# profi248/backuwup

Hardware: AMD Instinct MI355X
Metric: GB/s chunked+hashed+deduped (whole node, 1/2/4/8 GPU), bit-exact vs CPU (higher is better)
Workload: dtype u8

## Files before the change

backuwup_amd/csrc/bw_cdc.hip:

```cpp
#include "bw_device.h"
#include "bw_internal.h"

namespace bw {
#if BW_CLOCK_STAMPS
__device__ ClockLog* g_clk_cdc = nullptr;
void clock_log_register_cdc(void* log) { hipMemcpyToSymbol(HIP_SYMBOL(g_clk_cdc), &log, sizeof(log)); }
#endif


__constant__ uint64_t c_gear[256] = BW_GEAR_INIT;


__device__ __forceinline__ uint64_t gear_fetch(uint32_t word, uint32_t sel, uint32_t lane_off, const uint64_t* lds) {
    const uint32_t addr = __builtin_amdgcn_perm(word, lane_off, sel);
    return *(const uint64_t*)((const uint8_t*)lds + addr);
}

__device__ __forceinline__ void gear_step(uint64_t& h, uint32_t word, uint32_t sel, uint32_t lane_off,
                                          const uint64_t* lds) {
    h = (h << 1) + gear_fetch(word, sel, lane_off, lds);
}

#define BW_SEL(k) (0x0c0c0000u | ((4u + (k)) << 8))

__device__ __forceinline__ uint32_t mask_test(uint64_t h, uint32_t mlo, uint32_t mhi) {
    uint32_t r;
    const uint32_t t = (uint32_t)h & mlo;
    asm("v_and_or_b32 %0, %1, %2, %3" : "=v"(r) : "v"((uint32_t)(h >> 32)), "s"(mhi), "v"(t));
    return r;
}

__device__ __forceinline__ void record_hit(uint64_t pos, uint64_t h, const Masks& mk, uint32_t* s_cnt,
                                           uint64_t* s_slots) {
    const bool S = (h & mk.mask_s) == 0, L = (h & mk.mask_l) == 0;
    if (S || L) {
        uint32_t i = atomicAdd(s_cnt, 1u);
        if (i < (uint32_t)SCAN_CAP) s_slots[i] = pos | (S ? BW_CAND_S : 0) | (L ? BW_CAND_L : 0);
    }
}

__device__ __forceinline__ void hash_words(uint64_t& h, uint32_t& acc, const uint32_t (&ww)[16], uint32_t lane_off,
                                           const uint64_t* s_gear, uint32_t phi) {
#pragma unroll
    for (int i = 0; i < 16; i += 2) {
        uint64_t g[8];
#pragma unroll
        for (int q = 0; q < 8; q++) g[q] = gear_fetch(ww[i + q / 4], BW_SEL(q % 4), lane_off, s_gear);
#pragma unroll
        for (int q = 0; q < 8; q += 2) {
            h = (h << 1) + g[q];
            const uint32_t t0 = (uint32_t)(h >> 32) & phi;
            h = (h << 1) + g[q + 1];
            const uint32_t t1 = (uint32_t)(h >> 32) & phi;
            asm("v_min3_u32 %0, %1, %2, %3" : "=v"(acc) : "v"(acc), "v"(t0), "v"(t1));
        }
    }
}

__device__ __forceinline__ void stage_hash_step(uint4 r0, uint4 r1, uint4 r2, uint4 r3, uint8_t* wr,
                                                const uint8_t* rd, uint64_t& h, uint64_t at, uint32_t lane_off,
                                                const uint64_t* s_gear, uint32_t phi, uint32_t* cnt,
                                                uint64_t* slots) {
    *(uint4*)(wr) = r0;
    *(uint4*)(wr + 16 * STAGE_ROW) = r1;
    *(uint4*)(wr + 32 * STAGE_ROW) = r2;
    *(uint4*)(wr + 48 * STAGE_ROW) = r3;
    __builtin_amdgcn_wave_barrier();
    const uint4 v0 = *(const uint4*)(rd), v1 = *(const uint4*)(rd + 16), v2 = *(const uint4*)(rd + 32),
                v3 = *(const uint4*)(rd + 48);
    __builtin_amdgcn_wave_barrier();
    const uint32_t ww[16] = {v0.x, v0.y, v0.z, v0.w, v1.x, v1.y, v1.z, v1.w,
                             v2.x, v2.y, v2.z, v2.w, v3.x, v3.y, v3.z, v3.w};
    uint32_t acc = 0xffffffffu;
    hash_words(h, acc, ww, lane_off, s_gear, phi);
    if (__builtin_expect(acc == 0, 0)) {
        const uint32_t i = atomicAdd(cnt, 1u);
        if (i < (uint32_t)SCAN_CAP) slots[i] = at | BW_CAND_BLK;
    }
}

constexpr uint32_t TILE_OVF = 0x80000000u;

__device__ __forceinline__ void ovf_push(uint64_t t, uint32_t* ovf, uint64_t* ctr) {
    const uint64_t k = atomicAdd((unsigned long long*)&ctr[C_NOVF], 1ull);
    ovf[k] = (uint32_t)t;
}

__device__ __forceinline__ void refine_block(const uint8_t* __restrict__ data, uint64_t b, const uint64_t* s_gear,
                                             uint32_t lane, const Masks& mk, uint32_t* cnt, uint64_t* slots) {
    const uint32_t rep = (lane & 31) * 8;
    const uint64_t g0 = b >= 64 ? *(const uint64_t*)((const uint8_t*)s_gear + ((uint32_t)data[b - 64 + lane] << 8) + rep) : 0;
    const uint64_t g1 = *(const uint64_t*)((const uint8_t*)s_gear + ((uint32_t)data[b + lane] << 8) + rep);
    const uint64_t pre = bw_shfl64(bw_gear_scan(g0), 63);
    const uint64_t h = bw_gear_scan(g1) + ((pre << lane) << 1);
    record_hit(b + lane, h >> mk.pre_shift, mk, cnt, slots);
}


template <int BLOCK, int STRIP>
__global__ __launch_bounds__(BLOCK, 4) void k_scan(const uint8_t* __restrict__ data, uint64_t n_bytes,
                                                       uint64_t n_tiles, Masks mk,
                                                       uint32_t* __restrict__ tile_count,
                                                       uint64_t* __restrict__ tile_slots, uint32_t* __restrict__ ovf,
                                                       uint64_t* ctr) {
    constexpr int WAVES = BLOCK / 64;
    struct ScanLds {
        uint64_t gear[256 * GEAR_REP];
        uint8_t stage[WAVES][64 * STAGE_ROW];
        uint64_t slots[WAVES][SCAN_CAP];
        uint64_t flags[WAVES][SCAN_CAP];
        uint32_t cnt[WAVES], nflag[WAVES];
    };
    __shared__ __attribute__((aligned(16))) ScanLds lds;
    uint64_t* s_gear = lds.gear;
    uint8_t (*s_stage)[64 * STAGE_ROW] = lds.stage;
    uint64_t (*s_slots)[SCAN_CAP] = lds.slots;
    uint32_t* s_cnt = lds.cnt;
    for (int i = threadIdx.x; i < 256 * GEAR_REP; i += blockDim.x) s_gear[i] = c_gear[i / GEAR_REP] << mk.pre_shift;
    __syncthreads();
    const uint32_t lane = threadIdx.x & 63, wid = threadIdx.x >> 6;
    const uint32_t lane_off = (lane & 31) * 8;
    const uint32_t phi = mk.pre_hi;
    uint8_t* stage = s_stage[wid];
    uint32_t* cnt = &s_cnt[wid];
    uint64_t* slots = s_slots[wid];
    uint32_t* fcnt = &lds.nflag[wid];
    uint64_t* fslots = lds.flags[wid];
    const uint64_t nw = (uint64_t)gridDim.x * WAVES;

    for (uint64_t tile = (uint64_t)blockIdx.x * WAVES + wid; tile < n_tiles; tile += nw) {
#if BW_CLOCK_STAMPS
        ClockStamp clk((tile & 15) == 0 ? g_clk_cdc : nullptr, 0);
#endif
        if (lane == 0) { *cnt = 0; *fcnt = 0; }
        const uint64_t base = tile * (64ull * STRIP);
        const uint64_t ss = base + (uint64_t)lane * STRIP;
        uint64_t h = 0;
        if (base + (64ull * STRIP) <= n_bytes) {
            if (ss >= 64) {
                const uint4* wp = (const uint4*)(data + ss - 64);
                uint4 w[4];
#pragma unroll
                for (int i = 0; i < 4; i++) w[i] = wp[i];
#pragma unroll
                for (int i = 0; i < 4; i++) {
                    const uint32_t ww[4] = {w[i].x, w[i].y, w[i].z, w[i].w};
#pragma unroll
                    for (int j = 0; j < 4; j++)
#pragma unroll
                        for (int k = 0; k < 4; k++) gear_step(h, ww[j], BW_SEL(k), lane_off, s_gear);
                }
            }
            {
                const uint8_t* src = data + base + (uint64_t)(lane >> 2) * STRIP + (lane & 3) * 16;
                uint8_t* wr = stage + (lane >> 2) * STAGE_ROW + (lane & 3) * 16;
                const uint8_t* rd = stage + lane * STAGE_ROW;
                constexpr int STEPS = STRIP / SCAN_STEP;
                constexpr uint64_t JS = 16ull * STRIP;
#define BW_LOAD8(r, ds)                                                                          \
    do {                                                                                         \
        const uint8_t* s_ = src + (uint64_t)(ds) * (2 * SCAN_STEP);                              \
        _Pragma("unroll") for (int j = 0; j < 4; j++) {                                          \
            r[j] = *(const uint4*)(s_ + j * JS);                                                 \
            r[4 + j] = *(const uint4*)(s_ + SCAN_STEP + j * JS);                                 \
        }                                                                                        \
    } while (0)
                uint4 a[8], b[8];
                BW_LOAD8(a, 0);
#pragma unroll 1
                for (int ds = 0; ds < STEPS / 2; ds += 2) {
                    BW_LOAD8(b, ds + 1);
                    stage_hash_step(a[0], a[1], a[2], a[3], wr, rd, h, ss + (uint64_t)(2 * ds) * SCAN_STEP, lane_off,
                                    s_gear, phi, fcnt, fslots);
                    stage_hash_step(a[4], a[5], a[6], a[7], wr, rd, h, ss + (uint64_t)(2 * ds + 1) * SCAN_STEP,
                                    lane_off, s_gear, phi, fcnt, fslots);
                    BW_LOAD8(a, ds + 2 < STEPS / 2 ? ds + 2 : STEPS / 2 - 1);
                    stage_hash_step(b[0], b[1], b[2], b[3], wr, rd, h, ss + (uint64_t)(2 * ds + 2) * SCAN_STEP,
                                    lane_off, s_gear, phi, fcnt, fslots);
                    stage_hash_step(b[4], b[5], b[6], b[7], wr, rd, h, ss + (uint64_t)(2 * ds + 3) * SCAN_STEP,
                                    lane_off, s_gear, phi, fcnt, fslots);
                }
#undef BW_LOAD8
            }
        } else if (ss < n_bytes) {
            const uint64_t se = ss + STRIP < n_bytes ? ss + STRIP : n_bytes;
            for (uint64_t p = ss >= 64 ? ss - 64 : 0; p < se; p++) {
                h = (h << 1) + s_gear[(uint32_t)data[p] * GEAR_REP];
                if (p >= ss) record_hit(p, h >> mk.pre_shift, mk, cnt, slots);
            }
        }
        __builtin_amdgcn_wave_barrier();
        const uint32_t nf = __builtin_amdgcn_readfirstlane(*fcnt);
        if (nf <= (uint32_t)SCAN_CAP)
            for (uint32_t f = 0; f < nf; f++) refine_block(data, BW_CAND_POS(fslots[f]), s_gear, lane, mk, cnt, slots);
        __builtin_amdgcn_wave_barrier();
        if (lane == 0) {
            const uint32_t c = *cnt, n = c < (uint32_t)SCAN_CAP ? c : (uint32_t)SCAN_CAP;
            if (nf > (uint32_t)SCAN_CAP || c > (uint32_t)SCAN_CAP) ovf_push(tile, ovf, ctr);
            for (uint32_t i = 1; i < n; i++) {
                uint64_t v = slots[i];
                int k = (int)i - 1;
                while (k >= 0 && BW_CAND_POS(slots[k]) > BW_CAND_POS(v)) {
                    slots[k + 1] = slots[k];
                    k--;
                }
                slots[k + 1] = v;
            }
            tile_count[tile] = c;
            for (uint32_t i = 0; i < n; i++) tile_slots[tile * SCAN_CAP + i] = slots[i];
        }
        __builtin_amdgcn_wave_barrier();
    }
}

template <int BLOCK, int STRIP>
static void launch_scan_t(hipStream_t st, const uint8_t* data, uint64_t n_bytes, uint64_t n_tiles, const Masks& mk,
                          uint32_t* tile_count, uint64_t* tile_slots, uint32_t* ovf, uint64_t* ctr) {
    uint64_t grid = (n_tiles + BLOCK / 64 - 1) / (BLOCK / 64);
    const uint64_t cap = STRIP == SCAN_STRIP ? 512 : 1024;
    if (grid > cap) grid = cap;
    hipLaunchKernelGGL((k_scan<BLOCK, STRIP>), dim3((unsigned)grid), dim3(BLOCK), 0, st, data, n_bytes,
                       n_tiles, mk, tile_count, tile_slots, ovf, ctr);
}

bool launch_scan(hipStream_t st, const uint8_t* data, uint64_t n_bytes, uint64_t n_tiles, const Masks& mk,
                 uint32_t* tile_count, uint64_t* tile_slots, uint32_t* ovf, uint64_t* ctr, int waves) {
    if (!n_tiles) return true;
    const bool big = 64ull * SCAN_STRIP == 1ull << mk.tile_shift, small = 64ull * SCAN_STRIP_SMALL == 1ull << mk.tile_shift;
    if (!big && !small) return false;
#if BW_DIAG
    if (waves == 8) {
        if (big) launch_scan_t<512, SCAN_STRIP>(st, data, n_bytes, n_tiles, mk, tile_count, tile_slots, ovf, ctr);
        else launch_scan_t<512, SCAN_STRIP_SMALL>(st, data, n_bytes, n_tiles, mk, tile_count, tile_slots, ovf, ctr);
        return true;
    }
#endif
    (void)waves;
    if (big) launch_scan_t<SCAN_BLOCK, SCAN_STRIP>(st, data, n_bytes, n_tiles, mk, tile_count, tile_slots, ovf, ctr);
    else launch_scan_t<SCAN_BLOCK, SCAN_STRIP_SMALL>(st, data, n_bytes, n_tiles, mk, tile_count, tile_slots, ovf, ctr);
    return true;
}


template <int T>
__device__ __forceinline__ uint64_t block_excl_sum(uint64_t v, uint64_t* s, uint64_t* total) {
    s[threadIdx.x] = v;
    __syncthreads();
    for (int d = 1; d < T; d <<= 1) {
        uint64_t a = threadIdx.x >= (unsigned)d ? s[threadIdx.x - d] : 0;
        __syncthreads();
        s[threadIdx.x] += a;
        __syncthreads();
    }
    const uint64_t incl = s[threadIdx.x];
    if (total) *total = s[T - 1];
    __syncthreads();
    return incl - v;
}

template <int T>
__device__ __forceinline__ uint64_t block_excl_segmax(uint32_t f, uint64_t v, uint64_t* s, uint32_t* sf) {
    s[threadIdx.x] = v;
    sf[threadIdx.x] = f;
    __syncthreads();
    for (int d = 1; d < T; d <<= 1) {
        uint64_t a = 0;
        uint32_t af = 0;
        const bool has = threadIdx.x >= (unsigned)d;
        if (has) { a = s[threadIdx.x - d]; af = sf[threadIdx.x - d]; }
        __syncthreads();
        if (has && !sf[threadIdx.x]) { s[threadIdx.x] = a > s[threadIdx.x] ? a : s[threadIdx.x]; sf[threadIdx.x] = af; }
        __syncthreads();
    }
    uint64_t r = (threadIdx.x > 0) ? s[threadIdx.x - 1] : 0;
    __syncthreads();
    return r;
}

__device__ __forceinline__ bool last_block_done(uint64_t* done) {
    __shared__ bool last;
    __syncthreads();
    if (threadIdx.x == 0) {
        __threadfence();
        last = atomicAdd((unsigned long long*)done, 1ull) == gridDim.x - 1;
    }
    __syncthreads();
    if (last) {
        __threadfence();
        if (threadIdx.x == 0) *done = 0;
    }
    return last;
}

template <int T>
__device__ __forceinline__ uint64_t scan_totals(uint64_t* tot, uint64_t n, uint64_t* s) {
    const uint64_t per = (n + T - 1) / T, lo = threadIdx.x * per;
    const uint64_t hi = lo + per < n ? lo + per : n;
    uint64_t sum = 0;
    for (uint64_t i = lo; i < hi; i++) sum += tot[i];
    uint64_t total;
    uint64_t run = block_excl_sum<T>(sum, s, &total);
    for (uint64_t i = lo; i < hi; i++) {
        const uint64_t t = tot[i];
        tot[i] = run;
        run += t;
    }
    return total;
}


constexpr int BLK = 1024;

constexpr int RESCAN_THREADS = 256;

template <bool WRITE>
__device__ uint64_t rescan_tile(const uint8_t* __restrict__ data, uint64_t n_bytes, const Masks& mk, uint64_t tile,
                                uint64_t base, uint64_t* __restrict__ cand, uint64_t cap, const uint64_t* s_gear,
                                uint64_t* s_scan) {
    const uint64_t rs = (1ull << mk.tile_shift) / RESCAN_THREADS;
    const uint64_t ss = (tile << mk.tile_shift) + (uint64_t)threadIdx.x * rs;
    const uint64_t se = ss + rs < n_bytes ? ss + rs : n_bytes;
    uint64_t mine = 0, total = 0;
    for (int pass = 0; pass < (WRITE ? 2 : 1); pass++) {
        uint64_t h = 0, w = 0;
        if (pass == 1) w = base + block_excl_sum<RESCAN_THREADS>(mine, s_scan, nullptr);
        if (ss < n_bytes) {
            for (uint64_t p = ss >= 64 ? ss - 64 : 0; p < se; p++) {
                h = (h << 1) + s_gear[data[p]];
                if (p < ss) continue;
                const bool S = (h & mk.mask_s) == 0, L = (h & mk.mask_l) == 0;
                if (S || L) {
                    if (pass == 0) mine++;
                    else if (w < cap) cand[w++] = p | (S ? BW_CAND_S : 0) | (L ? BW_CAND_L : 0);
                }
            }
        }
    }
    if (!WRITE) block_excl_sum<RESCAN_THREADS>(mine, s_scan, &total);
    __syncthreads();
    return total;
}

template <bool WRITE>
__device__ void rescan_range(const uint8_t* __restrict__ data, uint64_t n_bytes, const Masks& mk,
                             const uint32_t* __restrict__ ovf, uint64_t novf, uint64_t t0, uint64_t t1,
                             uint32_t* __restrict__ tile_count, const uint64_t* __restrict__ off,
                             uint64_t* __restrict__ cand, uint64_t cap, uint64_t* s_gear, uint64_t* s_scan) {
    bool loaded = false;
    for (uint64_t k = 0; k < novf; k++) {
        const uint64_t tile = ovf[k];
        if (tile < t0 || tile >= t1) continue;
        if (!loaded) {
            for (int i = threadIdx.x; i < 256; i += blockDim.x) s_gear[i] = c_gear[i];
            __syncthreads();
            loaded = true;
        }
        const uint64_t total = rescan_tile<WRITE>(data, n_bytes, mk, tile, WRITE ? off[tile] : 0, cand, cap, s_gear,
                                                  s_scan);
        if (!WRITE && threadIdx.x == 0) tile_count[tile] = (uint32_t)total | TILE_OVF;
    }
    __syncthreads();
}

constexpr int TS_BLOCK = 256;

template <bool WRITE>
__global__ __launch_bounds__(RESCAN_THREADS) void k_rescan(const uint8_t* __restrict__ data, uint64_t n_bytes, Masks mk,
                                                            const uint32_t* __restrict__ ovf, uint32_t* __restrict__ cnt,
                                                            const uint64_t* __restrict__ off, uint64_t* __restrict__ cand,
                                                            uint64_t cap, const uint64_t* ctr) {
    __shared__ uint64_t s_gear[256], s_scan[RESCAN_THREADS];
    const uint64_t novf = ctr[C_NOVF];
    if (blockIdx.x >= novf) return;
    for (int i = threadIdx.x; i < 256; i += blockDim.x) s_gear[i] = c_gear[i];
    __syncthreads();
    for (uint64_t k = blockIdx.x; k < novf; k += gridDim.x) {
        const uint64_t tile = ovf[k];
        const uint64_t total = rescan_tile<WRITE>(data, n_bytes, mk, tile, WRITE ? off[tile] : 0, cand, cap, s_gear, s_scan);
        if (!WRITE && threadIdx.x == 0) cnt[tile] = (uint32_t)total | TILE_OVF;
    }
}

__global__ __launch_bounds__(TS_BLOCK) void k_tile_partial(const uint8_t* __restrict__ data, uint64_t n_bytes, Masks mk,
                                                           const uint32_t* __restrict__ ovf, uint32_t* __restrict__ cnt,
                                                           uint64_t n, uint64_t* __restrict__ off,
                                                           uint64_t* __restrict__ btot, uint64_t cap, uint64_t* ctr,
                                                           bool spread) {
    __shared__ uint64_t s[TS_BLOCK];
    __shared__ uint64_t s_gear[256];
    const uint64_t novf = spread ? 0 : ctr[C_NOVF];
    if (novf) {
        const uint64_t t0 = (uint64_t)blockIdx.x * 4 * TS_BLOCK, t1 = t0 + 4 * TS_BLOCK;
        rescan_range<false>(data, n_bytes, mk, ovf, novf, t0, t1 < n ? t1 : n, cnt, nullptr, nullptr, 0, s_gear, s);
    }
    const uint64_t i0 = ((uint64_t)blockIdx.x * TS_BLOCK + threadIdx.x) * 4;
    uint32_t c[4] = {0, 0, 0, 0};
    if (i0 + 4 <= n) {
        const uint4 v = *(const uint4*)(cnt + i0);
        c[0] = v.x; c[1] = v.y; c[2] = v.z; c[3] = v.w;
    } else {
        for (int k = 0; k < 4; k++) c[k] = i0 + k < n ? cnt[i0 + k] : 0;
    }
    for (int k = 0; k < 4; k++) c[k] &= ~TILE_OVF;
    const uint64_t sum = (uint64_t)c[0] + c[1] + c[2] + c[3];
    uint64_t total;
    uint64_t run = block_excl_sum<TS_BLOCK>(sum, s, &total);
    for (int k = 0; k < 4; k++)
        if (i0 + k < n) { off[i0 + k] = run; run += c[k]; }
    if (threadIdx.x == 0) btot[blockIdx.x] = total;
    if (!last_block_done(&ctr[C_DONE_TILES])) return;
    const uint64_t all = scan_totals<TS_BLOCK>(btot, gridDim.x, s);
    if (threadIdx.x == 0) {
        off[n] = all;
        ctr[C_NCAND] = all < cap ? all : cap;
        ctr[C_CANDTOTAL] = all;
        ctr[C_TRUNC] = BW_NONE;
    }
}

__global__ __launch_bounds__(256) void k_compact(const uint8_t* __restrict__ data, uint64_t n_bytes, Masks mk,
                                                 const uint32_t* __restrict__ ovf, const uint32_t* __restrict__ cnt,
                                                 const uint64_t* __restrict__ slots, uint64_t* __restrict__ off,
                                                 const uint64_t* __restrict__ bbase, uint64_t n_tiles,
                                                 uint64_t* __restrict__ cand, uint64_t cap, uint64_t* ctr, bool spread) {
    const uint64_t t = (uint64_t)blockIdx.x * blockDim.x + threadIdx.x;
    if (t < n_tiles) {
        const uint64_t o = off[t] + bbase[t / (4 * TS_BLOCK)];
        off[t] = o;
        const uint32_t c = cnt[t];
        if (o + (c & ~TILE_OVF) > cap)
            atomicMin((unsigned long long*)&ctr[C_TRUNC], (unsigned long long)(t << mk.tile_shift));
        if (!(c & TILE_OVF)) {
            for (uint32_t i = 0; i < c; i++)
                if (o + i < cap) cand[o + i] = slots[t * SCAN_CAP + i];
        }
    }
    const uint64_t novf = spread ? 0 : ctr[C_NOVF];
    if (novf) {
        __shared__ uint64_t s_gear[256], s_scan[RESCAN_THREADS];
        __syncthreads();
        const uint64_t t0 = (uint64_t)blockIdx.x * blockDim.x, t1 = t0 + blockDim.x;
        rescan_range<true>(data, n_bytes, mk, ovf, novf, t0, t1 < n_tiles ? t1 : n_tiles, nullptr, off, cand, cap,
                           s_gear, s_scan);
    }
}

void launch_compact(hipStream_t st, const uint8_t* data, uint64_t n_bytes, uint64_t n_tiles, const Masks& mk,
                    uint32_t* tile_count, uint64_t* tile_slots, uint64_t* tile_off, uint64_t* cand,
                    uint64_t cand_cap, uint32_t* ovf_list, uint64_t* ctr, uint64_t* btot) {
    if (!n_tiles) return;
    const uint64_t nb = (n_tiles + 4 * TS_BLOCK - 1) / (4 * TS_BLOCK);
    const double flagged = (double)(1ull << mk.tile_shift) / 64.0 *
                           (1.0 - pow(1.0 - ldexp(1.0, -__builtin_popcount(mk.pre_hi)), 64.0));
    const bool spread = flagged > SCAN_CAP / 2;
    const unsigned rb = (unsigned)std::min<uint64_t>(n_tiles, 2048);
    if (spread)
        hipLaunchKernelGGL(k_rescan<false>, dim3(rb), dim3(RESCAN_THREADS), 0, st, data, n_bytes, mk, ovf_list, tile_count,
                           nullptr, nullptr, 0, ctr);
    hipLaunchKernelGGL(k_tile_partial, dim3((unsigned)nb), dim3(TS_BLOCK), 0, st, data, n_bytes, mk, ovf_list,
                       tile_count, n_tiles, tile_off, btot, cand_cap, ctr, spread);
    hipLaunchKernelGGL(k_compact, dim3((unsigned)((n_tiles + 255) / 256)), dim3(256), 0, st, data, n_bytes, mk, ovf_list,
                       tile_count, tile_slots, tile_off, btot, n_tiles, cand, cand_cap, ctr, spread);
    if (spread)
        hipLaunchKernelGGL(k_rescan<true>, dim3(rb), dim3(RESCAN_THREADS), 0, st, data, n_bytes, mk, ovf_list, tile_count,
                           tile_off, cand, cand_cap, ctr);
}


struct Walker {
    const uint8_t* data;
    const uint64_t* cand;
    uint64_t ncand;
    const uint64_t* lgear;
    Masks mk;
    uint64_t trunc;
    uint64_t data_len;
};

__device__ uint64_t direct_scan(const Walker& W, uint64_t a, uint64_t hi, uint64_t c2a) {
    const int lane = bw_lane();
    BW_ASSERT(a >= 64 && a <= hi && hi <= W.data_len);
    uint64_t carry = bw_shfl64(bw_gear_scan(W.lgear[W.data[a - 64 + lane]]), 63);
    for (uint64_t b = a; b < hi; b += 64) {
        const uint64_t p = b + (uint64_t)lane;
        const bool valid = p < hi;
        const uint64_t g = valid ? W.lgear[W.data[p]] : 0;
        const uint64_t h = bw_gear_scan(g) + ((carry << lane) << 1);
        const uint64_t mask = p < c2a ? W.mk.mask_s : W.mk.mask_l;
        const uint64_t hb = __ballot(valid && (h & mask) == 0);
        if (hb) return b + (uint64_t)__builtin_ctzll(hb);
        carry = bw_shfl64(h, 63);
    }
    return BW_NONE;
}

__device__ uint64_t walk_next(const Walker& W, uint64_t s, uint64_t fe, uint64_t& cptr) {
    const int lane = bw_lane();
    BW_ASSERT(s < fe && fe <= W.data_len);
    const uint64_t rem = fe - s;
    if (rem <= W.mk.min) return fe;
    uint64_t center = W.mk.avg, remaining = rem;
    if (rem > W.mk.max) remaining = W.mk.max;
    else if (rem < center) center = rem;
    const uint64_t s0 = W.mk.s0, c2 = center & ~1ull, r2 = remaining & ~1ull;

    const uint64_t p = s0 + (uint64_t)lane;
    const bool valid = lane < 47 && p < r2;
    const uint64_t g = valid ? W.lgear[W.data[s + p]] : 0;
    const uint64_t h = bw_gear_scan(g);
    const uint64_t mask = p < c2 ? W.mk.mask_s : W.mk.mask_l;
    const uint64_t hb = __ballot(valid && (h & mask) == 0);
    if (hb) return s + s0 + (uint64_t)__builtin_ctzll(hb);

    const uint64_t lo = s + s0 + 47, hi = s + r2, c2a = s + c2;
    const uint64_t hc = hi < W.trunc ? hi : W.trunc;
    for (;;) {
        const uint64_t idx = cptr + (uint64_t)lane;
        const uint64_t c = idx < W.ncand ? W.cand[idx] : BW_NONE;
        const uint64_t pos = c == BW_NONE ? BW_NONE : BW_CAND_POS(c);
        const uint64_t below = __ballot(pos < lo);
        const bool match = pos >= lo && pos < hc && ((pos < c2a) ? (c & BW_CAND_S) != 0 : (c & BW_CAND_L) != 0);
        const uint64_t mb = __ballot(match);
        if (mb) {
            const uint64_t cut = bw_shfl64(pos, __builtin_ctzll(mb));
            cptr += (uint64_t)__popcll(below);
            BW_ASSERT(cut > s && cut < s + remaining && cptr <= W.ncand + 64);
            return cut;
        }
        if (__ballot(pos >= hc) != 0) {
            cptr += (uint64_t)__popcll(below);
            break;
        }
        cptr += 64;
    }
    if (hc < hi) {
        const uint64_t cut = direct_scan(W, lo > hc ? lo : hc, hi, c2a);
        if (cut != BW_NONE) return cut;
    }
    return s + remaining;
}

__device__ __forceinline__ void load_lgear(uint64_t* lg) {
    for (int i = threadIdx.x; i < 256; i += blockDim.x) lg[i] = c_gear[i];
    __syncthreads();
}


constexpr int WAVES_PER_BLOCK = 4;

__global__ __launch_bounds__(64 * WAVES_PER_BLOCK) void k_chains(Walker W, const uint64_t* __restrict__ tile_off,
                                                                 const uint64_t* ctr, const SegDesc* __restrict__ segs,
                                                                 uint64_t nseg, uint64_t* __restrict__ chains,
                                                                 uint32_t* __restrict__ chain_n,
                                                                 uint64_t* __restrict__ chain_cptr) {
    __shared__ uint64_t lg[256];
    load_lgear(lg);
    W.lgear = lg;
    W.ncand = ctr[C_NCAND];
    W.trunc = ctr[C_TRUNC];
    const uint64_t j = (uint64_t)blockIdx.x * WAVES_PER_BLOCK + threadIdx.x / 64;
    if (j >= nseg) return;
    const SegDesc sd = segs[j];
    uint64_t s = sd.start, cptr = tile_off[s >> W.mk.tile_shift];
    uint32_t n = 0;
    bool past = false;
    for (;;) {
        const uint64_t c = walk_next(W, s, sd.file_end, cptr);
        if (n < (uint32_t)CHAIN_CAP && bw_lane() == 0) chains[j * CHAIN_CAP + n] = c;
        n++;
        if (n > (uint32_t)CHAIN_CAP || c >= sd.file_end || (c >= sd.end && past)) break;
        past = c >= sd.end;
        s = c;
    }
    if (bw_lane() == 0) { chain_n[j] = n; chain_cptr[j] = cptr; }
}

__global__ __launch_bounds__(64 * WAVES_PER_BLOCK) void k_extend(Walker W, const uint64_t* ctr,
                                                                 const SegDesc* __restrict__ segs, uint64_t nseg,
                                                                 uint64_t* __restrict__ chains,
                                                                 uint32_t* __restrict__ chain_n,
                                                                 const uint64_t* __restrict__ chain_cptr,
                                                                 uint64_t* __restrict__ merge) {
    __shared__ uint64_t lg[256];
    load_lgear(lg);
    W.lgear = lg;
    W.ncand = ctr[C_NCAND];
    W.trunc = ctr[C_TRUNC];
    const uint64_t j = (uint64_t)blockIdx.x * WAVES_PER_BLOCK + threadIdx.x / 64;
    if (j >= nseg) return;
    const int lane = bw_lane();
    const SegDesc sd = segs[j];
    if (sd.last) { if (lane == 0) merge[j] = sd.file_end; return; }
    uint32_t n = chain_n[j];
    const uint32_t n1r = chain_n[j + 1];
    if (n > (uint32_t)CHAIN_CAP || n1r == 0) { if (lane == 0) merge[j] = BW_NONE; return; }
    const uint32_t n1 = n1r < (uint32_t)CHAIN_CAP ? n1r : (uint32_t)CHAIN_CAP;
    const uint64_t* c1 = chains + (j + 1) * CHAIN_CAP;
    const uint64_t v0 = (uint32_t)lane < n1 ? c1[lane] : BW_NONE;
    const uint64_t v1 = (uint32_t)lane + 64 < n1 ? c1[lane + 64] : BW_NONE;
    const uint64_t last1 = c1[n1 - 1];
    const uint64_t b1 = segs[j + 1].start;
    uint64_t e = chains[j * CHAIN_CAP + n - 1], cptr = chain_cptr[j], m = BW_NONE;
    for (;;) {
        if (e == b1 || __ballot(v0 == e || v1 == e) != 0) { m = e; break; }
        if (e >= last1 || n >= (uint32_t)CHAIN_CAP) break;
        e = walk_next(W, e, sd.file_end, cptr);
        if (lane == 0) chains[j * CHAIN_CAP + n] = e;
        n++;
    }
    if (lane == 0) { chain_n[j] = n; merge[j] = m; }
}

void launch_chains(hipStream_t st, const uint8_t* data, uint64_t data_len, const Masks& mk, const uint64_t* cand,
                   const uint64_t* tile_off, uint64_t* ctr, const SegDesc* segs, uint64_t nseg, uint64_t* chains,
                   uint32_t* chain_n, uint64_t* chain_cptr, uint64_t* merge, int force_serial) {
    if (!nseg || force_serial) return;
    Walker W{data, cand, 0, nullptr, mk, 0, data_len};
    const unsigned grid = (unsigned)((nseg + WAVES_PER_BLOCK - 1) / WAVES_PER_BLOCK);
    hipLaunchKernelGGL(k_chains, dim3(grid), dim3(64 * WAVES_PER_BLOCK), 0, st, W, tile_off, ctr, segs, nseg,
                       chains, chain_n, chain_cptr);
    hipLaunchKernelGGL(k_extend, dim3(grid), dim3(64 * WAVES_PER_BLOCK), 0, st, W, ctr, segs, nseg, chains,
                       chain_n, chain_cptr, merge);
}


__global__ __launch_bounds__(BLK) void k_resolve(const SegDesc* __restrict__ segs, uint64_t nseg,
                                                 const CFileDesc* __restrict__ cfiles, uint64_t ncf,
                                                 const uint64_t* __restrict__ chains,
                                                 const uint32_t* __restrict__ chain_n,
                                                 const uint64_t* __restrict__ merge, uint64_t* __restrict__ seg_M,
                                                 uint32_t* __restrict__ seg_cnt, uint32_t* __restrict__ cf_invalid,
                                                 int force_serial) {
    __shared__ uint64_t s_v[BLK];
    __shared__ uint32_t s_f[BLK];
    for (uint64_t f = threadIdx.x; f < ncf; f += BLK) cf_invalid[f] = 0;
    __syncthreads();
    const uint64_t per = (nseg + BLK - 1) / BLK, lo = threadIdx.x * per;
    const uint64_t hi = lo + per < nseg ? lo + per : nseg;
    uint32_t af = 0;
    uint64_t av = 0;
    for (uint64_t j = lo; j < hi; j++) {
        const bool head = cfiles[segs[j].cfile].first_seg == j;
        const uint64_t m = merge[j];
        if (head) { af = 1; av = m; } else { av = m > av ? m : av; }
    }
    uint64_t run = block_excl_segmax<BLK>(af, av, s_v, s_f);
    for (uint64_t j = lo; j < hi; j++) {
        const SegDesc sd = segs[j];
        const bool head = cfiles[sd.cfile].first_seg == j;
        if (head) run = 0;
        const uint64_t M = head ? sd.start : run;
        seg_M[j] = M;
        const uint64_t m = merge[j];
        run = m > run ? m : run;
        if (force_serial) { cf_invalid[sd.cfile] = 1; continue; }
    }
    __syncthreads();
    if (force_serial) return;
    for (uint64_t j = lo; j < hi; j++) {
        const SegDesc sd = segs[j];
        const uint32_t nr = chain_n[j];
        const uint64_t M = seg_M[j];
        const uint64_t R = sd.last ? sd.file_end : seg_M[j + 1];
        bool ok = nr <= (uint32_t)CHAIN_CAP && M != BW_NONE && R != BW_NONE;
        uint32_t cnt = 0;
        if (ok) {
            bool found = (M == sd.start);
            cnt = (M == sd.start && sd.start < R) ? 1 : 0;
            for (uint32_t k = 0; k < nr; k++) {
                const uint64_t e = chains[j * CHAIN_CAP + k];
                if (e == M) found = true;
                if (e >= M && e < R && e != sd.start) cnt++;
            }
            if (!sd.last && R > M) {
                bool reach = false;
                for (uint32_t k = 0; k < nr; k++) reach |= chains[j * CHAIN_CAP + k] == R;
                ok = reach;
            }
            ok = ok && found;
        }
        seg_cnt[j] = cnt;
        if (!ok) cf_invalid[sd.cfile] = 1;
    }
}

__global__ __launch_bounds__(64 * WAVES_PER_BLOCK) void k_fallback(Walker W, const uint64_t* __restrict__ tile_off,
                                                                   uint64_t* ctr, const CFileDesc* __restrict__ cfiles,
                                                                   uint64_t ncf, const uint32_t* __restrict__ cf_invalid,
                                                                   uint64_t* __restrict__ fb_starts,
                                                                   uint64_t* __restrict__ fb_count) {
    __shared__ uint64_t lg[256];
    load_lgear(lg);
    W.lgear = lg;
    W.ncand = ctr[C_NCAND];
    W.trunc = ctr[C_TRUNC];
    const uint64_t f = (uint64_t)blockIdx.x * WAVES_PER_BLOCK + threadIdx.x / 64;
    if (f >= ncf || !cf_invalid[f]) return;
    const CFileDesc cf = cfiles[f];
    uint64_t s = cf.start, cptr = tile_off[s >> W.mk.tile_shift], n = 0;
    while (s < cf.end) {
        if (bw_lane() == 0) fb_starts[cf.fb_off + n] = s;
        n++;
        s = walk_next(W, s, cf.end, cptr);
    }
    if (bw_lane() == 0) {
        fb_count[f] = n;
        atomicAdd((unsigned long long*)&ctr[C_NINVALID], 1ull);
    }
}

void launch_resolve(hipStream_t st, const uint8_t* data, uint64_t data_len, const Masks& mk, const uint64_t* cand,
                    const uint64_t* tile_off, uint64_t* ctr, const SegDesc* segs, uint64_t nseg,
                    const CFileDesc* cfiles, uint64_t ncf, const uint64_t* chains, const uint32_t* chain_n,
                    const uint64_t* merge, uint64_t* seg_M, uint32_t* seg_cnt, uint32_t* cf_invalid,
                    uint64_t* fb_starts, uint64_t* fb_count, int force_serial) {
    if (!nseg) return;
    hipLaunchKernelGGL(k_resolve, dim3(1), dim3(BLK), 0, st, segs, nseg, cfiles, ncf, chains, chain_n, merge, seg_M,
                       seg_cnt, cf_invalid, force_serial);
    Walker W{data, cand, 0, nullptr, mk, 0, data_len};
    const unsigned grid = (unsigned)((ncf + WAVES_PER_BLOCK - 1) / WAVES_PER_BLOCK);
    hipLaunchKernelGGL(k_fallback, dim3(grid), dim3(64 * WAVES_PER_BLOCK), 0, st, W, tile_off, ctr, cfiles, ncf,
                       cf_invalid, fb_starts, fb_count);
}


__device__ __forceinline__ uint64_t groups_of(uint64_t len, uint32_t gshift) {
    const uint64_t leaves = len == 0 ? 1 : (len + B3_LEAF_BYTES - 1) / B3_LEAF_BYTES;
    return (leaves + (1u << gshift) - 1) >> gshift;
}

template <bool WRITE>
__device__ void unit_blobs(const UnitDesc& u, const SegDesc* segs, const CFileDesc* cfiles, const uint64_t* chains,
                           const uint32_t* chain_n, const uint64_t* seg_M, const uint32_t* cf_invalid,
                           const uint64_t* fb_starts, const uint64_t* fb_count, BlobArrays b, uint64_t bbase,
                           uint64_t gbase, uint64_t& nb, uint64_t& ng) {
    nb = 0;
    ng = 0;
    auto emit = [&](uint64_t start, uint64_t end, uint32_t kind, uint64_t fend) {
        const uint64_t len = end - start;
        BW_ASSERT(start <= end && end <= fend && fend <= b.data_len);
        if (WRITE) {
            const uint64_t k = bbase + nb;
            BW_ASSERT(k < b.cap);
            b.start[k] = start;
            b.len[k] = len;
            b.goff[k] = gbase + ng;
            b.file[k] = u.file;
            b.kind[k] = kind;
            b.fend[k] = fend;
        }
        nb++;
        ng += groups_of(len, b.gshift);
    };
    if (u.kind == 0) { emit(u.start, u.start + u.len, 0, u.start + u.len); return; }
    const SegDesc sd = segs[u.seg];
    if (cf_invalid[u.cfile]) {
        const CFileDesc cf = cfiles[u.cfile];
        if (cf.first_seg != u.seg) return;
        const uint64_t n = fb_count[u.cfile];
        for (uint64_t i = 0; i < n; i++) {
            const uint64_t s = fb_starts[cf.fb_off + i];
            const uint64_t e = i + 1 < n ? fb_starts[cf.fb_off + i + 1] : cf.end;
            emit(s, e, 1, cf.end);
        }
        return;
    }
    const uint64_t M = seg_M[u.seg];
    const uint64_t R = sd.last ? sd.file_end : seg_M[u.seg + 1];
    if (M >= R) return;
    const uint32_t nr = chain_n[u.seg];
    uint64_t prev = BW_NONE;
    if (M == sd.start) prev = sd.start;
    for (uint32_t k = 0; k < nr; k++) {
        const uint64_t e = chains[u.seg * CHAIN_CAP + k];
        if (e < M || e == sd.start) continue;
        if (e >= R) break;
        if (prev != BW_NONE) emit(prev, e, 1, sd.file_end);
        prev = e;
    }
    if (prev != BW_NONE) emit(prev, R, 1, sd.file_end);
}

constexpr int AS_BLOCK = 256;
constexpr uint64_t AS_UNITS = AS_BLOCK;

__global__ __launch_bounds__(AS_BLOCK) void k_unit_count(const UnitDesc* __restrict__ units, uint64_t nunits,
                                                         const SegDesc* __restrict__ segs,
                                                         const CFileDesc* __restrict__ cfiles,
                                                         const uint64_t* __restrict__ chains,
                                                         const uint32_t* __restrict__ chain_n,
                                                         const uint64_t* __restrict__ seg_M,
                                                         const uint32_t* __restrict__ cf_invalid,
                                                         const uint64_t* __restrict__ fb_starts,
                                                         const uint64_t* __restrict__ fb_count, BlobArrays b,
                                                         uint64_t* __restrict__ ucb, uint64_t* __restrict__ ucg,
                                                         uint64_t* __restrict__ bt_b, uint64_t* __restrict__ bt_g,
                                                         uint64_t* ctr) {
    __shared__ uint64_t s[AS_BLOCK];
    const uint64_t u = (uint64_t)blockIdx.x * AS_BLOCK + threadIdx.x;
    uint64_t nb = 0, ng = 0;
    if (u < nunits)
        unit_blobs<false>(units[u], segs, cfiles, chains, chain_n, seg_M, cf_invalid, fb_starts, fb_count, b, 0, 0, nb,
                          ng);
    uint64_t tb, tg;
    const uint64_t rb = block_excl_sum<AS_BLOCK>(nb, s, &tb);
    const uint64_t rg = block_excl_sum<AS_BLOCK>(ng, s, &tg);
    if (u < nunits) {
        ucb[u] = rb;
        ucg[u] = rg;
    }
    if (threadIdx.x == 0) {
        bt_b[blockIdx.x] = tb;
        bt_g[blockIdx.x] = tg;
    }
    if (!last_block_done(&ctr[C_DONE_UNITS])) return;
    const uint64_t totb = scan_totals<AS_BLOCK>(bt_b, gridDim.x, s);
    const uint64_t totg = scan_totals<AS_BLOCK>(bt_g, gridDim.x, s);
    if (threadIdx.x == 0) {
        ctr[C_NBLOBS] = totb;
        ctr[C_NGROUPS] = totg;
        ctr[C_DEDUPN] = totb;
    }
}

__global__ __launch_bounds__(256) void k_unit_emit(const UnitDesc* __restrict__ units, uint64_t nunits,
                                                   const SegDesc* __restrict__ segs,
                                                   const CFileDesc* __restrict__ cfiles,
                                                   const uint64_t* __restrict__ chains,
                                                   const uint32_t* __restrict__ chain_n,
                                                   const uint64_t* __restrict__ seg_M,
                                                   const uint32_t* __restrict__ cf_invalid,
                                                   const uint64_t* __restrict__ fb_starts,
                                                   const uint64_t* __restrict__ fb_count, BlobArrays b,
                                                   const uint64_t* __restrict__ ucb, const uint64_t* __restrict__ ucg,
                                                   const uint64_t* __restrict__ bt_b,
                                                   const uint64_t* __restrict__ bt_g) {
    const uint64_t u = (uint64_t)blockIdx.x * blockDim.x + threadIdx.x;
    if (u >= nunits) return;
    const uint64_t bb = ucb[u] + bt_b[u / AS_UNITS], gb = ucg[u] + bt_g[u / AS_UNITS];
    uint64_t nb, ng;
    unit_blobs<true>(units[u], segs, cfiles, chains, chain_n, seg_M, cf_invalid, fb_starts, fb_count, b, bb, gb, nb,
                     ng);
}

void launch_assemble(hipStream_t st, uint64_t* ctr, const UnitDesc* units, uint64_t nunits, const SegDesc* segs,
                     const CFileDesc* cfiles, const uint64_t* chains, const uint32_t* chain_n, const uint64_t* seg_M,
                     const uint32_t* cf_invalid, const uint64_t* fb_starts, const uint64_t* fb_count, BlobArrays b,
                     uint64_t* ucnt, uint64_t* ubtot) {
    const uint64_t nblk = (nunits + AS_UNITS - 1) / AS_UNITS;
    uint64_t *ucb = ucnt, *ucg = ucnt + nunits, *bt_b = ubtot, *bt_g = ubtot + nblk + 1;
    if (!nunits) return;
    hipLaunchKernelGGL(k_unit_count, dim3((unsigned)nblk), dim3(AS_BLOCK), 0, st, units, nunits, segs, cfiles, chains,
                       chain_n, seg_M, cf_invalid, fb_starts, fb_count, b, ucb, ucg, bt_b, bt_g, ctr);
    hipLaunchKernelGGL(k_unit_emit, dim3((unsigned)((nunits + 255) / 256)), dim3(256), 0, st, units, nunits, segs,
                       cfiles, chains, chain_n, seg_M, cf_invalid, fb_starts, fb_count, b, ucb, ucg, bt_b, bt_g);
}


__global__ __launch_bounds__(256) void k_upload(const uint4* __restrict__ src, uint4* __restrict__ dst, uint64_t n16) {
    for (uint64_t i = (uint64_t)blockIdx.x * blockDim.x + threadIdx.x; i < n16; i += (uint64_t)gridDim.x * blockDim.x)
        dst[i] = src[i];
}

__global__ __launch_bounds__(64) void k_zero(uint64_t* __restrict__ p, uint32_t n) {
    for (uint32_t i = threadIdx.x; i < n; i += blockDim.x) p[i] = 0;
}

void launch_zero(hipStream_t st, uint64_t* p, uint32_t n) {
    hipLaunchKernelGGL(k_zero, dim3(1), dim3(64), 0, st, p, n);
}

void launch_upload(hipStream_t st, const void* host_src, void* dst, uint64_t bytes) {
    const uint64_t n16 = (bytes + 15) / 16;
    if (!n16) return;
    uint64_t grid = (n16 + 255) / 256;
    if (grid > 1024) grid = 1024;
    hipLaunchKernelGGL(k_upload, dim3((unsigned)grid), dim3(256), 0, st, (const uint4*)host_src, (uint4*)dst, n16);
}


__global__ __launch_bounds__(256) void k_cut_hash(const uint8_t* __restrict__ data, Masks mk,
                                                  const uint64_t* ctr, BlobArrays b) {
    const uint64_t k = (uint64_t)blockIdx.x * 4 + threadIdx.x / 64;
    if (k >= ctr[C_NBLOBS]) return;
    const int lane = bw_lane();
    if (b.kind[k] == 0) { if (lane == 0) b.ghash[k] = 0; return; }
    const uint64_t s = b.start[k], len = b.len[k], fe = b.fend[k];
    const uint64_t rem = fe - s;
    uint64_t out = 0;
    if (rem > mk.min) {
        const uint64_t remaining = rem > mk.max ? mk.max : rem;
        const uint64_t r2 = remaining & ~1ull;
        uint64_t p = BW_NONE;
        if (len == remaining) { if (r2 > mk.s0) p = r2 - 1; }
        else p = len;
        if (p != BW_NONE) {
            const uint64_t q = p - (uint64_t)lane;
            uint64_t term = 0;
            if ((uint64_t)lane <= p && q >= mk.s0) term = c_gear[data[s + q]] << lane;
            out = bw_wave_sum64(term);
            if ((p & 1) == 0) out <<= 1;
        }
    }
    if (lane == 0) b.ghash[k] = out;
}

void launch_cut_hash(hipStream_t st, const uint8_t* data, const Masks& mk, const uint64_t* ctr, BlobArrays b,
                     uint64_t max_blobs) {
    if (!max_blobs) return;
    hipLaunchKernelGGL(k_cut_hash, dim3((unsigned)((max_blobs + 3) / 4)), dim3(256), 0, st, data, mk, ctr, b);
}

}
```

backuwup_amd/csrc/bw_internal.h:

```cpp
#pragma once
#include <hip/hip_runtime.h>

#include "bw_plan.h"

#ifndef BW_DIAG
#define BW_DIAG 0
#endif

namespace bw {

constexpr int SCAN_BLOCK = 1024;
#ifndef BW_SCAN_CAP
#define BW_SCAN_CAP 16
#endif
constexpr int SCAN_STRIP_SMALL = SCAN_STRIP / 2;
constexpr uint64_t SCAN_SMALL_BYTES = 4ull << 30;
constexpr int SCAN_CAP = BW_SCAN_CAP;
constexpr int SCAN_STEP = 64;
constexpr int STAGE_ROW = SCAN_STEP + 16;
constexpr int GEAR_REP = 32;

enum Ctr : int {
    C_NCAND = 0,
    C_NOVF = 1,
    C_NBLOBS = 2,
    C_NGROUPS = 3,
    C_SEQBASE = 4,
    C_LOST = 5,
    C_NINVALID = 6,
    C_NUNIQUE = 7,
    C_CANDTOTAL = 8,
    C_DEDUPN = 9,
    C_TRUNC = 10,
    C_IX_OVF = 11,
    C_IX_LOGLEN = 12,
    C_IX_VALID = 13,
    C_DONE_TILES = 14,
    C_DONE_UNITS = 15,
    C_COUNT = 16
};
static_assert(SCAN_STRIP_SMALL % (4 * SCAN_STEP) == 0, "k_scan consumes four 64-byte steps per iteration");
static_assert(SCAN_STRIP % (4 * SCAN_STEP) == 0, "k_scan consumes four 64-byte steps per iteration");

struct BlobArrays {
    uint64_t* start;
    uint64_t* len;
    uint64_t* goff;
    uint32_t* file;
    uint32_t* kind;
    uint64_t* fend;
    uint64_t* ghash;
    uint64_t cap;
    uint64_t data_len;
    uint32_t* gdone = nullptr;
    uint32_t gshift = 2;
};

bool launch_scan(hipStream_t st, const uint8_t* data, uint64_t n_bytes, uint64_t n_tiles,
                 const Masks& mk, uint32_t* tile_count, uint64_t* tile_slots, uint32_t* ovf_list,
                 uint64_t* ctr, int waves );
void launch_compact(hipStream_t st, const uint8_t* data, uint64_t n_bytes, uint64_t n_tiles,
                    const Masks& mk, uint32_t* tile_count, uint64_t* tile_slots,
                    uint64_t* tile_off, uint64_t* cand, uint64_t cand_cap, uint32_t* ovf_list,
                    uint64_t* ctr, uint64_t* scratch );
void launch_chains(hipStream_t st, const uint8_t* data, uint64_t data_len, const Masks& mk, const uint64_t* cand,
                   const uint64_t* tile_off, uint64_t* ctr, const SegDesc* segs, uint64_t nseg,
                   uint64_t* chains, uint32_t* chain_n, uint64_t* chain_cptr, uint64_t* merge,
                   int force_serial);
void launch_resolve(hipStream_t st, const uint8_t* data, uint64_t data_len, const Masks& mk, const uint64_t* cand,
                    const uint64_t* tile_off, uint64_t* ctr, const SegDesc* segs, uint64_t nseg,
                    const CFileDesc* cfiles, uint64_t ncf, const uint64_t* chains,
                    const uint32_t* chain_n, const uint64_t* merge, uint64_t* seg_M,
                    uint32_t* seg_cnt, uint32_t* cf_invalid, uint64_t* fb_starts,
                    uint64_t* fb_count, int force_serial);
void launch_assemble(hipStream_t st, uint64_t* ctr, const UnitDesc* units, uint64_t nunits,
                     const SegDesc* segs, const CFileDesc* cfiles, const uint64_t* chains,
                     const uint32_t* chain_n, const uint64_t* seg_M, const uint32_t* cf_invalid,
                     const uint64_t* fb_starts, const uint64_t* fb_count, BlobArrays b,
                     uint64_t* ucnt , uint64_t* ubtot );
void launch_upload(hipStream_t st, const void* host_src, void* dst, uint64_t bytes);
void launch_zero(hipStream_t st, uint64_t* p, uint32_t n);
void launch_cut_hash(hipStream_t st, const uint8_t* data, const Masks& mk, const uint64_t* ctr,
                     BlobArrays b, uint64_t max_blobs);


enum { B3_LOADS_PREFETCH = 0, B3_LOADS_PAIRS = 1, B3_LOADS_LINES = 2 };
void launch_blake3(hipStream_t st, const uint8_t* data, const uint64_t* ctr, BlobArrays b,
                   uint64_t max_blobs, uint64_t max_groups, uint32_t* cv_buf,
                   uint32_t* cv_tmp , uint8_t* digests, int max_leaves,
                   hipEvent_t between , int loads,
                   hipStream_t upper ,
                   hipEvent_t leaf_done = nullptr ,
                   hipEvent_t mark = nullptr );
void launch_b3_calib(hipStream_t st, uint32_t n_blocks, uint32_t blocks_per_lane, uint32_t* sink, uint64_t* stamps);
uint32_t b3_calib_blocks_per_cu();
enum DState : int { D_LOGLEN = 0, D_NUNIQUE = 1, D_LOST = 2, D_BUCKET_OVF = 3, D_DONE = 4, D_COUNT = 5 };
void launch_table_clear(hipStream_t st, uint64_t* table, uint64_t cap);
void launch_dedup(hipStream_t st, uint64_t* table, uint64_t cap, uint8_t* log, uint64_t* dstate,
                  const uint8_t* digests, const uint64_t* n_dev, uint64_t n_host, uint64_t max_n,
                  uint8_t* is_dup);
void launch_rehash(hipStream_t st, uint64_t* table, uint64_t cap, const uint8_t* log,
                   const uint64_t* dstate, uint64_t max_n);
void launch_partition(hipStream_t st, const uint8_t* digests, uint64_t n, uint32_t n_owners,
                      uint8_t* out, uint64_t* perm, uint64_t* counts_dev);
void launch_scatter(hipStream_t st, const uint8_t* verdict, const uint64_t* perm, uint64_t n,
                    uint8_t* is_dup);
void launch_bucket_partition(hipStream_t st, const uint8_t* digests, const uint64_t* n_dev, uint64_t max_n,
                             uint32_t n_owners, uint64_t cap, uint8_t* out, uint64_t* perm, uint64_t* counts,
                             uint64_t* blk, uint64_t* err);
void launch_bucket_gather(hipStream_t st, const uint8_t* buckets, const uint64_t* counts, uint32_t n_src, uint64_t cap,
                          uint8_t* out, uint64_t* n_out);
void launch_bucket_expand(hipStream_t st, const uint64_t* counts, uint32_t n_src, uint64_t cap, const uint8_t* v_in,
                          uint8_t* v_out);
void launch_bucket_scatter(hipStream_t st, const uint8_t* verdict, const uint64_t* perm, const uint64_t* counts,
                           uint32_t n_owners, uint64_t cap, uint8_t* is_dup, uint8_t* packed = nullptr);
void launch_pack(hipStream_t st, uint64_t* ctr, BlobArrays b, const uint64_t* file_start,
                 const uint8_t* digests, const uint8_t* is_dup, uint8_t* out, uint64_t max_blobs,
                 const uint64_t* dstate, uint8_t* host = nullptr, uint64_t host_n = 0);
void launch_index_snapshot(hipStream_t st, const uint64_t* dstate, uint64_t* ctr);
void launch_owner_partition(hipStream_t st, const uint8_t* digests, const uint64_t* n_dev, uint64_t max_n,
                            uint32_t n_owners, uint8_t* out, uint64_t* perm, uint64_t* msg, uint64_t* blk);
void launch_copy_u64(hipStream_t st, const uint64_t* src, uint64_t* dst, uint32_t n);
void launch_owner_scatter(hipStream_t st, const uint8_t* verdict, const uint64_t* perm, uint64_t n, uint8_t* is_dup,
                          uint8_t* packed);

constexpr uint32_t PIECE_BLOCKS = 8192;
constexpr int SEAL_THREADS = 1024;

struct SealItem {
    uint64_t src_off, len, dst_off, piece0;
    uint32_t nonce[3];
    uint32_t info_len;
    uint8_t info[56];
    uint32_t raw_len, wd;
};

struct SealKey {
    uint32_t rk[60];
    uint32_t H[4], E0[4], HP[4], H64[4];
    uint32_t P[6][4];
    uint32_t R1[4];
};

struct SealPads {
    uint32_t istate[8], ostate[8];
};
void seal_pads(const uint8_t prk[32], SealPads* pads);
uint64_t seal_pieces(uint64_t len);
void seal_fill_item(SealItem* it, uint64_t src_off, uint64_t len, uint64_t dst_off, uint64_t piece0,
                    const uint8_t nonce[12], const uint8_t* info, uint32_t info_len);
void launch_seal(hipStream_t st, bool dec, bool framed, const uint8_t* src, uint8_t* dst, const SealItem* items,
                 uint64_t n, const SealPads& pads, SealKey* keys, uint64_t n_pieces, uint32_t* parts, uint8_t* ok);
uint32_t zstd_window_descriptor(uint64_t raw_len);

constexpr int GF_ROW_TILE = 8;
constexpr uint32_t GF_WAVE_BYTES = 2048;
constexpr uint32_t GF_GRID_BLOCKS = 1024;

int ctx_device(const bw_ctx* c);
int batch_set_exchange_range(bw_ctx* c, uint64_t ticket, uint64_t first, uint64_t n);
uint8_t* message_stage(bw_ctx* c, size_t bytes);
int hash_messages(bw_ctx* c, const uint8_t* staged, uint64_t total, const uint64_t* offs, const uint64_t* lens,
                  uint64_t n, bool dedup, uint8_t* hashes, uint8_t* dup);

int comm_rank(const bw_comm* c);
int comm_world(const bw_comm* c);
int comm_device(const bw_comm* c);
bool comm_failed(const bw_comm* c);
void*& comm_exq(bw_comm* c);
uint64_t comm_now_ns();
int comm_wait_event(bw_comm* c, hipEvent_t ev, std::string& err);
int comm_poll(bw_comm* c, hipEvent_t ev, uint64_t since_ns, bool* ready, std::string& err);
int comm_counts(bw_comm* c, const uint64_t* d_send, uint64_t* d_recv, uint64_t* h, hipStream_t st, bool* now,
                std::string& err);
int comm_all_to_allv(bw_comm* c, const void* d_send, const uint64_t* scnt, void* d_recv, const uint64_t* rcnt,
                     uint64_t elem, uint64_t pad, hipStream_t st, std::string& err);
int comm_allgather2(bw_comm* c, const uint64_t mine[2], uint64_t* all, std::string& err);
int exchange_progress(bw_comm* c, const void* until);
void exchange_drain(bw_comm* c);

constexpr uint32_t ZSTD_BLOCK = 131072;
constexpr uint32_t ZSTD_STRIDE = ZSTD_BLOCK + 3;

struct PackBlob {
    uint8_t hash[32];
    uint8_t nonce[12];
    uint32_t kind;
    uint64_t sealed_len;
    uint64_t section_off;
    uint64_t hdr_off;
    uint64_t nonce_off;
};

struct PackFileDesc {
    uint64_t hdr_off, count, out_off, header_len;
};

void launch_pack_meta(hipStream_t st, const PackBlob* blobs, uint64_t n, const PackFileDesc* files, uint64_t n_files,
                      uint8_t* hdr, uint8_t* out);
void launch_index_parse(hipStream_t st, const uint8_t* pt, const uint64_t* pt_off, const uint64_t* pt_len,
                        uint64_t n_files, uint64_t* parsed);
void launch_index_gather(hipStream_t st, const uint8_t* pt, const uint64_t* file_rec0, const uint64_t* file_src,
                         uint64_t n_files, uint64_t n_rec, uint8_t* digests, uint8_t* records);

struct ZstdWork;
void zstd_work_free(ZstdWork* w);
void zstd_work_limits(ZstdWork*& w, uint64_t max_slots, uint64_t max_bytes);
void zstd_work_copy_limits(ZstdWork*& dst, const ZstdWork* src);
int zstd_compress(hipStream_t st, ZstdWork*& w, const uint8_t* d_src, const uint64_t* src_off, const uint64_t* src_len,
                  uint64_t n, uint8_t* d_dst, const uint64_t* dst_off, uint64_t* frame_len, std::string& err);

}
```

Measured before the change: 1944.

## Replace per-lane 64-byte warmup hash with deferred neighbor-lane head recompute

Drops the serial 64-byte gear-hash warmup each lane ran before its strip. Instead each lane starts its hash cold, saves the first bytes of its strip to LDS and registers, and after the main loop takes the previous lane's final hash through a shuffle. It then rehashes only the head words to detect boundary candidates in the overlap region. The first block's hits are masked, tile-start blocks are refined unconditionally, and the logic that keeps results bit-exact is more intricate. The cost is extra LDS, extra registers, and one unconditional refine_block per tile.

```diff
diff --git a/backuwup_amd/csrc/bw_cdc.hip b/backuwup_amd/csrc/bw_cdc.hip
--- a/backuwup_amd/csrc/bw_cdc.hip
+++ b/backuwup_amd/csrc/bw_cdc.hip
@@ -14,11 +14,6 @@
 __device__ __forceinline__ uint64_t gear_fetch(uint32_t word, uint32_t sel, uint32_t lane_off, const uint64_t* lds) {
     const uint32_t addr = __builtin_amdgcn_perm(word, lane_off, sel);
     return *(const uint64_t*)((const uint8_t*)lds + addr);
-}
-
-__device__ __forceinline__ void gear_step(uint64_t& h, uint32_t word, uint32_t sel, uint32_t lane_off,
-                                          const uint64_t* lds) {
-    h = (h << 1) + gear_fetch(word, sel, lane_off, lds);
 }
 
 #define BW_SEL(k) (0x0c0c0000u | ((4u + (k)) << 8))
@@ -39,10 +34,11 @@
     }
 }
 
-__device__ __forceinline__ void hash_words(uint64_t& h, uint32_t& acc, const uint32_t (&ww)[16], uint32_t lane_off,
-                                           const uint64_t* s_gear, uint32_t phi) {
+template <int NW, bool FIRST>
+__device__ __forceinline__ void hash_words(uint64_t& h, uint32_t& acc, const uint32_t (&ww)[NW], uint32_t lane_off,
+                                           const uint64_t* s_gear, uint32_t phi, bool head) {
 #pragma unroll
-    for (int i = 0; i < 16; i += 2) {
+    for (int i = 0; i < NW; i += 2) {
         uint64_t g[8];
 #pragma unroll
         for (int q = 0; q < 8; q++) g[q] = gear_fetch(ww[i + q / 4], BW_SEL(q % 4), lane_off, s_gear);
@@ -54,13 +50,15 @@
             const uint32_t t1 = (uint32_t)(h >> 32) & phi;
             asm("v_min3_u32 %0, %1, %2, %3" : "=v"(acc) : "v"(acc), "v"(t0), "v"(t1));
         }
-    }
-}
-
-__device__ __forceinline__ void stage_hash_step(uint4 r0, uint4 r1, uint4 r2, uint4 r3, uint8_t* wr,
+        if (FIRST && i + 2 == HEAD_WORDS && head) acc = 0xffffffffu;
+    }
+}
+
+template <bool FIRST>
+__device__ __forceinline__ bool stage_hash_step(uint4 r0, uint4 r1, uint4 r2, uint4 r3, uint8_t* wr,
                                                 const uint8_t* rd, uint64_t& h, uint64_t at, uint32_t lane_off,
                                                 const uint64_t* s_gear, uint32_t phi, uint32_t* cnt,
-                                                uint64_t* slots) {
+                                                uint64_t* slots, bool head, uint64_t* hx, uint32_t (&hd)[HEAD_REGS]) {
     *(uint4*)(wr) = r0;
     *(uint4*)(wr + 16 * STAGE_ROW) = r1;
     *(uint4*)(wr + 32 * STAGE_ROW) = r2;
@@ -71,12 +69,20 @@
     __builtin_amdgcn_wave_barrier();
     const uint32_t ww[16] = {v0.x, v0.y, v0.z, v0.w, v1.x, v1.y, v1.z, v1.w,
                              v2.x, v2.y, v2.z, v2.w, v3.x, v3.y, v3.z, v3.w};
+    if (FIRST && head) {
+        *(uint4*)(const_cast<uint8_t*>(rd) + SCAN_STEP) = v0;
+        *hx = (uint64_t)v1.x | (uint64_t)v1.y << 32;
+#pragma unroll
+        for (int i = 0; i < HEAD_REGS; i++) hd[i] = ww[HEAD_WORDS - HEAD_REGS + i];
+    }
     uint32_t acc = 0xffffffffu;
-    hash_words(h, acc, ww, lane_off, s_gear, phi);
-    if (__builtin_expect(acc == 0, 0)) {
+    hash_words<16, FIRST>(h, acc, ww, lane_off, s_gear, phi, head);
+    const bool hit = acc == 0;
+    if (__builtin_expect(hit, 0)) {
         const uint32_t i = atomicAdd(cnt, 1u);
         if (i < (uint32_t)SCAN_CAP) slots[i] = at | BW_CAND_BLK;
     }
+    return hit;
 }
 
 constexpr uint32_t TILE_OVF = 0x80000000u;
@@ -109,6 +115,7 @@
         uint8_t stage[WAVES][64 * STAGE_ROW];
         uint64_t slots[WAVES][SCAN_CAP];
         uint64_t flags[WAVES][SCAN_CAP];
+        uint64_t head[WAVES][64];
         uint32_t cnt[WAVES], nflag[WAVES];
     };
     __shared__ __attribute__((aligned(16))) ScanLds lds;
@@ -126,6 +133,7 @@
     uint64_t* slots = s_slots[wid];
     uint32_t* fcnt = &lds.nflag[wid];
     uint64_t* fslots = lds.flags[wid];
+    uint64_t* hx = &lds.head[wid][lane];
     const uint64_t nw = (uint64_t)gridDim.x * WAVES;
 
     for (uint64_t tile = (uint64_t)blockIdx.x * WAVES + wid; tile < n_tiles; tile += nw) {
@@ -136,21 +144,10 @@
         const uint64_t base = tile * (64ull * STRIP);
         const uint64_t ss = base + (uint64_t)lane * STRIP;
         uint64_t h = 0;
-        if (base + (64ull * STRIP) <= n_bytes) {
-            if (ss >= 64) {
-                const uint4* wp = (const uint4*)(data + ss - 64);
-                uint4 w[4];
-#pragma unroll
-                for (int i = 0; i < 4; i++) w[i] = wp[i];
-#pragma unroll
-                for (int i = 0; i < 4; i++) {
-                    const uint32_t ww[4] = {w[i].x, w[i].y, w[i].z, w[i].w};
-#pragma unroll
-                    for (int j = 0; j < 4; j++)
-#pragma unroll
-                        for (int k = 0; k < 4; k++) gear_step(h, ww[j], BW_SEL(k), lane_off, s_gear);
-                }
-            }
+        const bool full = base + (64ull * STRIP) <= n_bytes;
+        uint64_t first_hit = 0;
+        if (full) {
+            uint32_t hd[HEAD_REGS];
             {
                 const uint8_t* src = data + base + (uint64_t)(lane >> 2) * STRIP + (lane & 3) * 16;
                 uint8_t* wr = stage + (lane >> 2) * STAGE_ROW + (lane & 3) * 16;
@@ -170,17 +167,32 @@
 #pragma unroll 1
                 for (int ds = 0; ds < STEPS / 2; ds += 2) {
                     BW_LOAD8(b, ds + 1);
-                    stage_hash_step(a[0], a[1], a[2], a[3], wr, rd, h, ss + (uint64_t)(2 * ds) * SCAN_STEP, lane_off,
-                                    s_gear, phi, fcnt, fslots);
-                    stage_hash_step(a[4], a[5], a[6], a[7], wr, rd, h, ss + (uint64_t)(2 * ds + 1) * SCAN_STEP,
-                                    lane_off, s_gear, phi, fcnt, fslots);
+                    const bool f = stage_hash_step<true>(a[0], a[1], a[2], a[3], wr, rd, h,
+                                                         ss + (uint64_t)(2 * ds) * SCAN_STEP, lane_off, s_gear, phi,
+                                                         fcnt, fslots, ds == 0, hx, hd);
+                    if (ds == 0) first_hit = __ballot(f);
+                    stage_hash_step<false>(a[4], a[5], a[6], a[7], wr, rd, h, ss + (uint64_t)(2 * ds + 1) * SCAN_STEP,
+                                           lane_off, s_gear, phi, fcnt, fslots, false, hx, hd);
                     BW_LOAD8(a, ds + 2 < STEPS / 2 ? ds + 2 : STEPS / 2 - 1);
-                    stage_hash_step(b[0], b[1], b[2], b[3], wr, rd, h, ss + (uint64_t)(2 * ds + 2) * SCAN_STEP,
-                                    lane_off, s_gear, phi, fcnt, fslots);
-                    stage_hash_step(b[4], b[5], b[6], b[7], wr, rd, h, ss + (uint64_t)(2 * ds + 3) * SCAN_STEP,
-                                    lane_off, s_gear, phi, fcnt, fslots);
+                    stage_hash_step<false>(b[0], b[1], b[2], b[3], wr, rd, h, ss + (uint64_t)(2 * ds + 2) * SCAN_STEP,
+                                           lane_off, s_gear, phi, fcnt, fslots, false, hx, hd);
+                    stage_hash_step<false>(b[4], b[5], b[6], b[7], wr, rd, h, ss + (uint64_t)(2 * ds + 3) * SCAN_STEP,
+                                           lane_off, s_gear, phi, fcnt, fslots, false, hx, hd);
                 }
 #undef BW_LOAD8
+            }
+            {
+                uint64_t hh = bw_shfl_up64(h, 1);
+                const uint4 p = *(const uint4*)(stage + lane * STAGE_ROW + SCAN_STEP);
+                const uint64_t x = *hx;
+                const uint32_t ww[HEAD_WORDS] = {p.x, p.y, p.z, p.w, (uint32_t)x, (uint32_t)(x >> 32),
+                                                 hd[0], hd[1], hd[2], hd[3], hd[4], hd[5]};
+                uint32_t acc = 0xffffffffu;
+                hash_words<HEAD_WORDS, false>(hh, acc, ww, lane_off, s_gear, phi, false);
+                if (__builtin_expect(acc == 0 && lane != 0 && !((first_hit >> lane) & 1), 0)) {
+                    const uint32_t i = atomicAdd(fcnt, 1u);
+                    if (i < (uint32_t)SCAN_CAP) fslots[i] = ss | BW_CAND_BLK;
+                }
             }
         } else if (ss < n_bytes) {
             const uint64_t se = ss + STRIP < n_bytes ? ss + STRIP : n_bytes;
@@ -191,8 +203,10 @@
         }
         __builtin_amdgcn_wave_barrier();
         const uint32_t nf = __builtin_amdgcn_readfirstlane(*fcnt);
-        if (nf <= (uint32_t)SCAN_CAP)
+        if (nf <= (uint32_t)SCAN_CAP) {
+            if (full && !(first_hit & 1)) refine_block(data, base, s_gear, lane, mk, cnt, slots);
             for (uint32_t f = 0; f < nf; f++) refine_block(data, BW_CAND_POS(fslots[f]), s_gear, lane, mk, cnt, slots);
+        }
         __builtin_amdgcn_wave_barrier();
         if (lane == 0) {
             const uint32_t c = *cnt, n = c < (uint32_t)SCAN_CAP ? c : (uint32_t)SCAN_CAP;
diff --git a/backuwup_amd/csrc/bw_internal.h b/backuwup_amd/csrc/bw_internal.h
--- a/backuwup_amd/csrc/bw_internal.h
+++ b/backuwup_amd/csrc/bw_internal.h
@@ -18,6 +18,8 @@
 constexpr int SCAN_CAP = BW_SCAN_CAP;
 constexpr int SCAN_STEP = 64;
 constexpr int STAGE_ROW = SCAN_STEP + 16;
+constexpr int HEAD_WORDS = 12;
+constexpr int HEAD_REGS = 6;
 constexpr int GEAR_REP = 32;
 
 enum Ctr : int {
```

Result: no change. 1939 (median of 2 runs) (-0.3%).
